# SandeepaInduwaraSamaranayake/SwinVox

Measured on AMD Instinct MI355X. Metric: views/sec fwd+bwd SwinVox-T 224^2, 32^3 voxel, n_views=8, higher is better.
Workload: dtype bf16; 1 GPU; SwinVox-T full pipeline (ResNet50[:layer3] || Swin multi-stage, cross-view attention, decoder, merger, refiner), fwd+2xBCE+bwd, train mode, B=64 samples x V=8 views of 224x224 per GPU; global_batch=64, n_views=8, images_per_gpu=512, parallelism=single GPU, launch=eager (one host launch per kernel, three streams)

## Files before the change

### include/swinvox_hip.h

```cpp
#ifndef SWINVOX_HIP_H
#define SWINVOX_HIP_H
#include <stddef.h>
#include <stdint.h>

#ifdef __cplusplus
extern "C" {
#endif

#define SV_OK 0
#define SV_ERR_INVALID (-1)
#define SV_ERR_LAUNCH (-2)

enum { SV_ACT_NONE = 0, SV_ACT_RELU = 1, SV_ACT_GELU = 2, SV_ACT_LRELU = 3 };
#define SV_BN_SLOTS 16
enum { SV_MATH_F32 = 0, SV_MATH_BF16 = 1, SV_MATH_FP8 = 2, SV_MATH_FP8_FULL = 3 };
enum { SV_F32 = 0, SV_BF16 = 1 };

const char* sv_last_error(void);
int sv_version(void);

typedef struct sv_geom {
  int N;
  int Di, Hi, Wi;
  int Do, Ho, Wo;
// ... 44 lines not shown
                        int act_dtype, void* stream);
int sv_linear_fp8_dgrad_supported(int N, int K, const sv_epilogue* e, int math, int act_dtype);
int sv_linear_fp8_wgrad(const void* dyt, const float* sdc, const void* xt, const float* sxc, float* dw, int M, int N, int K, int ldw, int splits,
                        void* stream);
long long sv_linear_fp8_bwd_launches(int which);
int sv_quant_rows_mx_e4m3(const void* src, int src_dtype, int rows, int K, int ld, void* dst_q, int Kp, void* scales_u8, void* stream);
int sv_linear_mxfp8(const void* xq, const void* xs, const void* wq, const void* ws, void* out, int M, int K, int N, const sv_epilogue* e,
                    void* q_out, void* qs_out, int act_dtype, void* stream);
long long sv_linear_mxfp8_launches(void);
long long sv_quant_rows_mx_launches(void);
int sv_quant_cols_mx_e4m3(const void* src, int src_dtype, int M, int C, int ld, void* dst_q, int Mp, void* scales_u8, float* colsum, void* stream);
int sv_linear_mxfp8_dgrad(const void* dq, const void* ds, const void* wtq, const void* wts, void* dx, int M, int N, int K, const sv_epilogue* e,
                          int act_dtype, void* stream);
size_t sv_linear_mxfp8_wgrad_workspace_floats(int M, int N, int K, int splits);
int sv_linear_mxfp8_wgrad(const void* dyt, const void* dys, const void* xt, const void* xs, float* dw, int M, int N, int K, int ldw, int splits,
                          float* workspace, void* stream);
long long sv_linear_mxfp8_bwd_launches(int which);
long long sv_quant_cols_mx_launches(void);
int sv_mx_rows_to_cols(const void* xq, int Kp, const void* xs, int M, int K, void* dst_q, int Mp, void* scales_u8, void* stream);
long long sv_mx_rows_to_cols_launches(void);
int sv_quant_rows_cols_mx_e4m3(const void* src, int src_dtype, int M, int N, int ld, void* row_q, int Np, void* row_s, void* col_q, int Mp,
                               void* col_s, float* colsum, void* stream);
long long sv_quant_rows_cols_mx_launches(void);
int sv_stencil3_fwd(const void* x, int ldx, int cin_load, int groups, const void* w_bf16, int ntiles16,
                    const float* bias, void* out, int ldc, int col_off, int cout, const void* residual, int ldr,
                    double* stats, int I, int D, int H, int W, long long x_plane_stride, long long out_plane_stride, int act_dtype,
                    void* stream);
size_t sv_stencil3_wgrad_workspace_floats(int cout, int cin);
int sv_stencil3_wgrad(const void* x, int ldx, int cin_load, int groups, const void* dy, int lddy, int cout_load,
                      float* dw, float* dbias, float* workspace, int cout, int cin, int c_stride, int c_valid, int I, int D, int H, int W,
                      long long x_plane_stride, int act_dtype, void* stream);
int sv_tconv4s2_fwd(const void* x, const void* w_packed, const float* bias, void* out, double* stats, int I, int D, int H, int W,
                    int cin, int cout, void* stream);
int sv_pack_weight(const float* src, void* dst, int A, int B, int T, int swap, int pad_to, int out_dtype, void* stream);
typedef struct sv_pack_desc {
  const float* src; void* dst;
  int A, B, T, swap, rows_out, inner_out, block0, reserved;
} sv_pack_desc;
int sv_pack_weights_block_elems(void);
int sv_pack_weights(const sv_pack_desc* descs_dev, int n, int total_blocks, int out_dtype, void* stream);
int sv_colsum(const void* x, int rows, int cols, int ld, float* out, int accumulate, int act_dtype, void* stream);
int sv_cast(const void* src, int src_dtype, void* dst, int dst_dtype, long long n, void* stream);

int sv_layernorm_fwd(const void* x, const float* gamma, const float* beta, void* y, float* mean, float* rstd,
                     long long rows, int C, float eps, int merge_H, int merge_W, int act_dtype, void* stream);
int sv_layernorm_quant_fwd(const void* x, const float* gamma, const float* beta, void* y, float* mean, float* rstd,
                           void* q, int Kp, float* scales, long long rows, int C, float eps, int merge_H, int merge_W,
                           int act_dtype, void* stream);
long long sv_layernorm_quant_launches(void);
int sv_layernorm_quant_mx_fwd(const void* x, const float* gamma, const float* beta, void* y, float* mean, float* rstd,
                              void* q, int Kp, void* scales_u8, long long rows, int C, float eps,
                              int merge_H, int merge_W, int act_dtype, void* stream);
long long sv_layernorm_quant_mx_launches(void);
size_t sv_layernorm_bwd_workspace_floats(int C);
int sv_layernorm_bwd(const void* dy, const void* x, const float* gamma, const float* mean, const float* rstd,
                     void* dx, float* dgamma, float* dbeta, float* workspace, long long rows, int C, int merge_H, int merge_W,
                     int accumulate_dx, int act_dtype, void* stream);
size_t sv_ln_image_workspace_floats(int I, int L);
int sv_ln_image_fwd(const void* x, const float* w, const float* b, void* y, float* meanrstd, float* workspace,
                    int I, int L, float eps, float drop_p, uint32_t seed, const uint32_t* seed_epoch, int act_dtype, void* stream);
int sv_ln_image_bwd(const void* dy, const void* x, const float* w, const float* meanrstd, void* dx, float* dw,
                    float* db, double* sums_ws , int I, int L, float drop_p, uint32_t seed,
                    const uint32_t* seed_epoch, int act_dtype, void* stream);
int sv_bn_stats(const void* x, long long M, int C, int ld, double* sums, int act_dtype, void* stream);
int sv_bn_finalize(const double* sums, long long count, const float* gamma, const float* beta, float* running_mean,
                   float* running_var, float momentum, float eps, int training, float* scale, float* shift,
// ... 127 lines not shown
```

### swinvox_amd/csrc/stencil.hip

```cpp
#include "common.h"
#include <map>
#include <mutex>
#include <type_traits>

namespace sv {

constexpr int TZ = 4, TY = 8, TX = 8;
constexpr int HZ = TZ + 2, HY = TY + 2, HX = TX + 2;
constexpr int HPOS = HZ * HY * HX;
constexpr int NVOX = TZ * TY * TX;
typedef __attribute__((address_space(3))) bf16x4 lds_bf16x4_t;

__device__ __forceinline__ bf16x4 to_bf16x4(float4 v) {
  bf16x4 b;
  b[0] = (__bf16)v.x; b[1] = (__bf16)v.y; b[2] = (__bf16)v.z; b[3] = (__bf16)v.w;
  return b;
}
__device__ __forceinline__ bf16x4 to_bf16x4(bf16x4 v) { return v; }

__device__ __forceinline__ int xcd_first_tile() {
  const int n = gridDim.x, b = blockIdx.x;
  return (n & 7) == 0 ? (b & 7) * (n >> 3) + (b >> 3) : b;
}

// ... 420 lines not shown
          for (int j = 0; j < 4; ++j) o[j] = (__bf16)(acc[j] + bias4[j]);
          const int oz = 2 * jz + az, oy = 2 * jy + ay, ox = 2 * xx + ax;
          *reinterpret_cast<bf16x4*>(Os + ((oz * 8 + oy) * 16 + ox) * 8 + lg * 4) = o;
        }
      }
    }
    __syncthreads();
#pragma unroll
    for (int k = 0; k < 4; ++k) {
      const int v = tid + 256 * k;
      const int ox = v & 15, oy = (v >> 4) & 7, oz = v >> 7;
      const bf16x8 o = *reinterpret_cast<const bf16x8*>(Os + v * 8);
      const size_t pos = (((size_t)img * (2 * p.D) + 2 * z0 + oz) * (2 * p.H) + 2 * y0 + oy) * (2 * p.W) + 2 * x0 + ox;
      *reinterpret_cast<bf16x8*>(p.out + pos * 8) = o;
      if (p.stats) {
#pragma unroll
        for (int c = 0; c < 8; ++c) { const double f = (double)(float)o[c]; st1[c] += f; st2[c] += f * f; }
      }
    }
    __syncthreads();
  }
  if (p.stats) {
#pragma unroll
    for (int c = 0; c < 8; ++c) {
      float a = (float)st1[c], b2 = (float)st2[c];
      a = wave_sum(a); b2 = wave_sum(b2);
      if (lane == 0) { red[wave][c] = a; red[wave][8 + c] = b2; }
    }
    __syncthreads();
    if (tid < 16 && (tid & 7) < p.cout) {
      const float v = red[0][tid] + red[1][tid] + red[2][tid] + red[3][tid];
      double* st = p.stats + (size_t)(blockIdx.x % SV_BN_SLOTS) * 2 * p.cout;
      atomicAdd(st + (tid >> 3) * p.cout + (tid & 7), (double)v);
    }
  }
}

}

using namespace sv;

static int resident_per_cu(const void* kernel, int threads = 256) {
  static std::mutex mu;
  static std::map<const void*, int> cache;
  std::lock_guard<std::mutex> lk(mu);
  auto it = cache.find(kernel);
  if (it != cache.end()) return it->second;
  int n = 0;
  if (hipOccupancyMaxActiveBlocksPerMultiprocessor(&n, kernel, threads, 0) != hipSuccess || n < 1) { (void)hipGetLastError(); n = 1; }
  cache[kernel] = n;
  return n;
}

static int stencil_check(int I, int D, int H, int W) {
  SV_REQUIRE(I > 0 && D % 8 == 0 && H % TY == 0 && W % TX == 0, "stencil3: grid %dx%dx%d must be a multiple of the 8x8x8 brick", D, H, W);
  return SV_OK;
}

#define SV_STENCIL_LAUNCH(GG, NTT, VV)                                                                                     \
  do {                                                                                                                    \
    constexpr int nthr = StencilBrickF<GG>::NTHR;                                                                         \
    const int nt_ = I * (D / StencilBrickF<GG>::TZV) * (H / TY) * (W / TX);                                               \
    a.ntiles = nt_;                                                                                                       \
    const int resident = 256 * resident_per_cu((const void*)stencil3_fwd_kernel<GG, NTT, AT, VV>, nthr);                  \
    hipLaunchKernelGGL((stencil3_fwd_kernel<GG, NTT, AT, VV>), dim3(nt_ < resident ? nt_ : resident), dim3(nthr), 0, s, a); \
  } while (0)
// ... 35 lines not shown

extern "C" size_t sv_stencil3_wgrad_workspace_floats(int cout, int cin) { return (size_t)WG_SLOTS * cout * cin * 27; }

extern "C" int sv_stencil3_wgrad(const void* x, int ldx, int cin_load, int groups, const void* dy, int lddy, int cout_load,
                                 float* dw, float* dbias, float* workspace, int cout, int cin, int c_stride, int c_valid, int I, int D, int H,
                                 int W, long long x_plane_stride, int act_dtype, void* stream) {
  SV_REQUIRE(x && dy && dw, "stencil3_wgrad: null argument");
  SV_REQUIRE(x_plane_stride >= 0 && x_plane_stride % 4 == 0 && (!x_plane_stride || cin_load % ldx == 0), "stencil3_wgrad: bad plane stride");
  SV_REQUIRE_ACT(act_dtype);
  if (int rc = stencil_check(I, D, H, W)) return rc;
  SV_REQUIRE(cin_load % 4 == 0 && cin_load <= 16 * groups && ldx % 4 == 0 && cout_load % 4 == 0 && cout_load <= 16 && lddy % 4 == 0,
             "stencil3_wgrad: bad channel layout");
  SV_REQUIRE(cout > 0 && cout <= 16 && cin > 0 && c_stride > 0 && c_valid > 0, "stencil3_wgrad: bad channel counts");
  SV_REQUIRE((((uintptr_t)x | (uintptr_t)dy) & (act_dtype == SV_BF16 ? 7 : 15)) == 0, "stencil3_wgrad: operands must be aligned to 4 elements");
  SV_REQUIRE(groups == 1 || groups == 3, "stencil3_wgrad: unsupported groups=%d", groups);
    const int ntiles = I * (D / (groups == 3 ? StencilBrick<3>::TZV : StencilBrick<1>::TZV)) * (H / TY) * (W / TX);
  hipStream_t s = (hipStream_t)stream;
  SV_DISPATCH_ACT(act_dtype,
    const int per_cu = groups == 1 ? resident_per_cu((const void*)stencil3_wgrad_kernel<1, AT>, StencilBrick<1>::NTHR)
                                   : resident_per_cu((const void*)stencil3_wgrad_kernel<3, AT>, StencilBrick<3>::NTHR);
    const int resident = 256 * per_cu;
    const int blocks = ntiles < resident ? ntiles : resident;
    StencilWArgsT<AT> a{static_cast<const AT*>(x), ldx, cin_load, x_plane_stride, static_cast<const AT*>(dy), lddy, cout_load, dw, workspace, dbias, cout, cin, c_stride, c_valid,
                        I, D, H, W, ntiles};
    if (groups == 1) hipLaunchKernelGGL((stencil3_wgrad_kernel<1, AT>), dim3(blocks), dim3(StencilBrick<1>::NTHR), 0, s, a);
    else hipLaunchKernelGGL((stencil3_wgrad_kernel<3, AT>), dim3(blocks), dim3(StencilBrick<3>::NTHR), 0, s, a););
  if (workspace) hipLaunchKernelGGL(stencil_wgrad_fold_kernel, dim3(cdiv(cout * cin * 27, 256)), dim3(256), 0, s, workspace, dw, cout * cin * 27);
  return check_launch("sv_stencil3_wgrad");
}

extern "C" int sv_tconv4s2_fwd(const void* x, const void* w_packed, const float* bias, void* out, double* stats, int I, int D, int H, int W,
                               int cin, int cout, void* stream) {
  SV_REQUIRE(x && w_packed && out && I > 0, "tconv4s2_fwd: null argument");
  SV_REQUIRE(cin == 32 && cout > 0 && cout <= 8, "tconv4s2_fwd: built for 32 input and <= 8 output channels (got %d -> %d)", cin, cout);
  SV_REQUIRE(D % T4_JZ == 0 && H % T4_JY == 0 && W % T4_JX == 0, "tconv4s2_fwd: input grid %dx%dx%d must be a multiple of the 4x4x8 brick", D, H, W);
  SV_REQUIRE((((uintptr_t)x | (uintptr_t)w_packed | (uintptr_t)out) & 15) == 0, "tconv4s2_fwd: operands must be 16-byte aligned");
  TConv4Args a{static_cast<const __bf16*>(x), static_cast<const __bf16*>(w_packed), bias, static_cast<__bf16*>(out), stats, cout, I, D, H, W,
               I * (D / T4_JZ) * (H / T4_JY) * (W / T4_JX)};
  const int blocks = a.nbricks < 512 ? a.nbricks : 512;
  hipLaunchKernelGGL(tconv4s2_fwd_kernel, dim3(blocks), dim3(256), 0, (hipStream_t)stream, a);
  return check_launch("sv_tconv4s2_fwd");
}
```

### swinvox_amd/hip.py

```python
from __future__ import annotations

import ctypes as C
import os
import threading

import torch

_HERE = os.path.dirname(os.path.abspath(__file__))
LIB_PATH = os.environ.get("SV_HIP_LIB") or os.path.join(_HERE, "libswinvox_hip.so")

ACT_NONE, ACT_RELU, ACT_GELU, ACT_LRELU = 0, 1, 2, 3
MATH_F32, MATH_BF16, MATH_FP8, MATH_FP8_FULL = 0, 1, 2, 3
F32, BF16 = 0, 1


class Geom(C.Structure):
    _fields_ = [(n, C.c_int) for n in ("N", "Di", "Hi", "Wi", "Do", "Ho", "Wo", "Ci", "Co", "kd", "kh", "kw",
                                        "sd", "sh", "sw", "pd", "ph", "pw", "ldi")]


class Epilogue(C.Structure):
    _fields_ = [("bias", C.c_void_p), ("residual", C.c_void_p), ("ldr", C.c_int), ("row_scale", C.c_void_p),
                ("rows_per_scale", C.c_int), ("pre_act", C.c_void_p), ("stats", C.c_void_p), ("act", C.c_int),
                ("slope", C.c_float), ("act_grad_src", C.c_void_p), ("act_grad_kind", C.c_int), ("ldc", C.c_int),
# ... 27 lines not shown
    "sv_conv_gather": (_I, [_P, _P, _P, C.POINTER(Geom), C.POINTER(Epilogue), _I]),
    "sv_tconv_gather": (_I, [_P, _P, _P, C.POINTER(Geom), C.POINTER(Epilogue), _I]),
    "sv_conv_gather_is_wide": (_I, None, [_P, _P, _P, C.POINTER(Geom), C.POINTER(Epilogue), _I, _I]),
    "sv_conv_wgrad_is_wide": (_I, None, [_P, _I, _P, C.POINTER(Geom), _I, _I, _I]),
    "sv_conv_wgrad_workspace_floats": (C.c_size_t, None, [C.POINTER(Geom)]),
    "sv_conv_wgrad": (_I, [_P, _I, _P, _P, C.POINTER(Geom), _I, _P, _P, _I]),
    "sv_quant_rows_e4m3": (_I, [_P, _I, _I, _I, _I, _P, _I, _P]),
    "sv_linear_fp8": (_I, [_P, _P, _P, _P, _P, _I, _I, _I, C.POINTER(Epilogue)]),
    "sv_linear_fp8_supported": (_I, None, [_I, _I, C.POINTER(Epilogue), _I, _I]),
    "sv_linear_fp8_launches": (_L, None),
    "sv_quant_cols_e4m3": (_I, [_P, _I, _I, _I, _I, _P, _I, _P, _P]),
    "sv_linear_fp8_dgrad": (_I, [_P, _P, _P, _P, _P, _I, _I, _I, C.POINTER(Epilogue)]),
    "sv_linear_fp8_dgrad_supported": (_I, None, [_I, _I, C.POINTER(Epilogue), _I, _I]),
    "sv_linear_fp8_wgrad": (_I, [_P, _P, _P, _P, _P, _I, _I, _I, _I, _I]),
    "sv_linear_fp8_bwd_launches": (_L, None, [_I]),
    "sv_quant_rows_mx_e4m3": (_I, [_P, _I, _I, _I, _I, _P, _I, _P]),
    "sv_linear_mxfp8": (_I, [_P, _P, _P, _P, _P, _I, _I, _I, C.POINTER(Epilogue), _P, _P]),
    "sv_linear_mxfp8_launches": (_L, None),
    "sv_quant_rows_mx_launches": (_L, None),
    "sv_quant_cols_mx_e4m3": (_I, [_P, _I, _I, _I, _I, _P, _I, _P, _P]),
    "sv_linear_mxfp8_dgrad": (_I, [_P, _P, _P, _P, _P, _I, _I, _I, C.POINTER(Epilogue)]),
    "sv_linear_mxfp8_wgrad_workspace_floats": (C.c_size_t, None, [_I, _I, _I, _I]),
    "sv_linear_mxfp8_wgrad": (_I, [_P, _P, _P, _P, _P, _I, _I, _I, _I, _I, _P]),
    "sv_linear_mxfp8_bwd_launches": (_L, None, [_I]),
    "sv_quant_cols_mx_launches": (_L, None),
    "sv_mx_rows_to_cols": (_I, [_P, _I, _P, _I, _I, _P, _I, _P]),
    "sv_mx_rows_to_cols_launches": (_L, None),
    "sv_quant_rows_cols_mx_e4m3": (_I, [_P, _I, _I, _I, _I, _P, _I, _P, _P, _I, _P, _P]),
    "sv_quant_rows_cols_mx_launches": (_L, None),
    "sv_stencil3_fwd": (_I, [_P, _I, _I, _I, _P, _I, _P, _P, _I, _I, _I, _P, _I, _P, _I, _I, _I, _I, _L, _L]),
    "sv_stencil3_wgrad_workspace_floats": (C.c_size_t, None, [_I, _I]),
    "sv_stencil3_wgrad": (_I, [_P, _I, _I, _I, _P, _I, _I, _P, _P, _P, _I, _I, _I, _I, _I, _I, _I, _I, _L]),
    "sv_tconv4s2_fwd": (_I, [_P, _P, _P, _P, _P, _I, _I, _I, _I, _I, _I]),
    "sv_pack_weight": (_I, [_P, _P, _I, _I, _I, _I, _I, _I]),
    "sv_pack_weights_block_elems": (_I, None),
    "sv_pack_weights": (_I, [_P, _I, _I, _I]),
    "sv_colsum": (_I, [_P, _I, _I, _I, _P, _I]),
    "sv_cast": (_I, [_P, _I, _P, _I, _L]),
    "sv_layernorm_fwd": (_I, [_P, _P, _P, _P, _P, _P, _L, _I, _F, _I, _I]),
    "sv_layernorm_quant_fwd": (_I, [_P, _P, _P, _P, _P, _P, _P, _I, _P, _L, _I, _F, _I, _I]),
    "sv_layernorm_quant_launches": (_L, None),
    "sv_layernorm_quant_mx_fwd": (_I, [_P, _P, _P, _P, _P, _P, _P, _I, _P, _L, _I, _F, _I, _I]),
    "sv_layernorm_quant_mx_launches": (_L, None),
    "sv_layernorm_bwd_workspace_floats": (C.c_size_t, None, [_I]),
    "sv_layernorm_bwd": (_I, [_P, _P, _P, _P, _P, _P, _P, _P, _P, _L, _I, _I, _I, _I]),
    "sv_bn_bwd_workspace_doubles": (C.c_size_t, None, [_I]),
    "sv_ln_image_workspace_floats": (C.c_size_t, None, [_I, _I]),
    "sv_ln_image_fwd": (_I, [_P, _P, _P, _P, _P, _P, _I, _I, _F, _F, _U, _P]),
    "sv_ln_image_bwd": (_I, [_P, _P, _P, _P, _P, _P, _P, _P, _I, _I, _F, _U, _P]),
    "sv_bn_stats": (_I, [_P, _L, _I, _I, _P]),
    "sv_bn_finalize": (_I, [_P, _L, _P, _P, _P, _P, _F, _F, _I, _P, _P, _P, _P, _I]),
    "sv_scale_shift_act": (_I, [_P, _I, _P, _P, _P, _I, _P, _I, _L, _I, _I, _F]),
    "sv_bn_bwd": (_I, [_P, _I, _P, _I, _P, _I, _P, _P, _P, _L, _I, _I, _F, _I, _P, _I, _P, _I, _P, _P, _P, _P, _P]),
    "sv_bn_signs_supported": (_I, None, [_I]),
    "sv_scale_shift_act_signs": (_I, [_P, _I, _P, _P, _P, _I, _P, _I, _L, _I, _I, _F, _P]),
    "sv_bn_bwd_signs": (_I, [_P, _I, _P, _P, _I, _P, _P, _P, _L, _I, _I, _F, _I, _P, _I, _P, _I, _P, _P, _P]),
    "sv_window_attention_fwd": (_I, [_P, _P, _P, _I, _I, _I, _I, _I, _I, _I]),
    "sv_window_attention_fwd_mxq": (_I, [_P, _P, _P, _I, _I, _I, _I, _I, _I, _I, _P, _I, _P]),
    "sv_window_attention_bwd_workspace_floats": (C.c_size_t, None, [_I]),
    "sv_window_attention_windows_per_group": (_I, None, [_I, _I, _I, _I, _I, _I]),
    "sv_window_attention_bwd": (_I, [_P, _P, _P, _P, _P, _P, _I, _I, _I, _I, _I, _I, _I]),
    "sv_stem_space_to_depth": (_I, [_P, _P, _I]),
    "sv_bn_act_maxpool_fwd": (_I, [_P, _P, _P, _P, _P, _I, _I, _I, _I, _I, _F]),
    "sv_bn_maxpool_bwd": (_I, [_P, _P, _P, _P, _P, _P, _P, _P, _I, _I, _I, _I, _I, _F, _I, _P, _P, _P, _P]),
    "sv_bn_act_maxpool3d_fwd": (_I, [_P, _P, _P, _P, _P, _I, _I, _I, _I, _I, _I, _F]),
    "sv_bn_maxpool3d_bwd": (_I, [_P, _P, _P, _P, _P, _P, _P, _P, _I, _I, _I, _I, _I, _I, _F, _I, _P, _P, _P, _P]),
# ... 200 lines not shown
```

### swinvox_amd/ops.py

```python
from __future__ import annotations

import ctypes as C
import threading
from dataclasses import dataclass
from typing import Optional, Tuple

import torch

from . import hip
from .hip import ACT_GELU, ACT_LRELU, ACT_NONE, ACT_RELU, Epilogue, Geom, call, ptr

_STATE = {"math": hip.MATH_F32, "store": torch.float32}


class _CallContext(threading.local):
    packs = None
    arena = None
    awg = None
    bn_tick = None
    dyq = None


_CTX = _CallContext()
BN_SLOTS = 16
BN_BWD_SLOTS, LN_BWD_SLOTS = 16, 32


def set_math(mode: str) -> None:
    _STATE["math"] = {"f32": hip.MATH_F32, "fp32": hip.MATH_F32, "bf16": hip.MATH_BF16}[mode]
    if _STATE["math"] == hip.MATH_F32:
        set_storage("f32")


def get_math() -> str:
    return "bf16" if _STATE["math"] == hip.MATH_BF16 else "f32"
# ... 122 lines not shown

    def pack_fwd(self, w: torch.Tensor) -> torch.Tensor:
        return self._pack(w, "f")

    def pack_dgrad(self, w: torch.Tensor) -> torch.Tensor:
        return self._pack(w, "d")

    def _geom(self, n, gathered_grid, produced_grid, ci, co, ldi) -> Geom:
        return Geom(n, *gathered_grid, *produced_grid, ci, co, *self.k, *self.s, *self.p, ldi)

    def _traced(self, name, n, in_grid, *args):
        tr = hip.TRACE
        if tr is None or name not in tr.names:
            return call(name, *args)
        og = self.out_grid(in_grid)
        if self.transposed:
            pairs = n * in_grid[0] * in_grid[1] * in_grid[2] * self.taps
        else:
            pairs = n * og[0] * og[1] * og[2] * self.taps
        flops = 2.0 * pairs * self.cin * self.cout
        nin, nout = n * in_grid[0] * in_grid[1] * in_grid[2], n * og[0] * og[1] * og[2]
        esz = 2.0 if _STATE["store"] == torch.bfloat16 else 4.0
        nbytes = esz * (nin * self.cin + nout * self.cout) + 4.0 * self.taps * self.cin * self.cout
        tr.begin(name, flops, nbytes, tag=f"n={n} grid={in_grid} cin={self.cin} cout={self.cout} k={self.k} s={self.s} t={int(self.transposed)}")
        call(name, *args)
        tr.end()

    def _halo_tconv(self, in_grid, ldi, ldc, epi) -> bool:
        return (self.transposed and self.k == (4, 4, 4) and self.s == (2, 2, 2) and self.p == (1, 1, 1) and self.cin == 32
                and self.cin_mem == 32 and self.cout == 8 and _STATE["store"] == torch.bfloat16 and _STATE["math"] != hip.MATH_F32
                and ldi in (None, 32) and ldc in (None, 8) and not (set(epi) - {"bias", "stats"})
                and in_grid[0] % 4 == 0 and in_grid[1] % 4 == 0 and in_grid[2] % 8 == 0)

    def forward(self, x, n, in_grid, w_packed, out, *, ldi=None, ldc=None, **epi):
        og = self.out_grid(in_grid)
        if isinstance(w_packed, torch.nn.Parameter) or w_packed.dtype != _STATE["store"]:
            w_packed = self.pack_fwd(w_packed)
        if self._halo_tconv(in_grid, ldi, ldc, epi):
            self._traced("sv_tconv4s2_fwd", n, in_grid, ptr(x), ptr(w_packed), ptr(epi.get("bias")), ptr(out), ptr(epi.get("stats")),
                         n, *in_grid, self.cin, self.cout)
            return og
        g = self._geom(n, in_grid, og, self.cin_mem, self.cout, ldi or self.cin_mem)
        e = _epilogue(ldc or self.cout, **epi)
        self._traced("sv_tconv_gather" if self.transposed else "sv_conv_gather", n, in_grid, ptr(x), ptr(w_packed), ptr(out),
                     C.byref(g), C.byref(e), _STATE["math"])
        return og

    def dgrad(self, dy, n, in_grid, w_dgrad, dx, *, lddy=None, lddx=None, **epi):
        og = self.out_grid(in_grid)
        g = self._geom(n, og, in_grid, self.cout_mem, self.cin, lddy or self.cout_mem)
        e = _epilogue(lddx or self.cin_mem, **epi)
        dense = self.taps == 1 and self.s == (1, 1, 1) and self.p == (0, 0, 0)
        self._traced("sv_conv_gather" if (self.transposed or dense) else "sv_tconv_gather", n, in_grid, ptr(dy), ptr(w_dgrad), ptr(dx),
                     C.byref(g), C.byref(e), _STATE["math"])

    def wgrad(self, dy, x, n, in_grid, dw, *, lddy=None, ldx=None, db=None, async_ok=True):
        aw = _CTX.awg
        if aw is not None and async_ok:
            cur = torch.cuda.current_stream()
            aw.stream.wait_stream(cur)
            aw.held.append((dy, x))
            with torch.cuda.stream(aw.stream):
                self._wgrad(dy, x, n, in_grid, dw, lddy, ldx, db)
            return
        self._wgrad(dy, x, n, in_grid, dw, lddy, ldx, db)

    def _wgrad(self, dy, x, n, in_grid, dw, lddy, ldx, db):
        og = self.out_grid(in_grid)
        if self.transposed:
            g = self._geom(n, og, in_grid, self.cout_mem, self.cin, lddy or self.cout_mem)
            ws = fempty(self.cin * self.taps * self.cout_mem, like=dw) if self.taps > 1 else None
            self._traced("sv_conv_wgrad", n, in_grid, ptr(x), ldx or self.cin_mem, ptr(dy), ptr(dw), C.byref(g), self.cout, ptr(ws),
                         None, _STATE["math"])
            if db is not None:
                colsum(dy, n * og[0] * og[1] * og[2], self.cout, lddy or self.cout_mem, db)
        else:
            g = self._geom(n, in_grid, og, self.cin_mem, self.cout, ldx or self.cin_mem)
            ws = fempty(self.cout * self.taps * self.cin_mem, like=dw) if self.taps > 1 else None
            self._traced("sv_conv_wgrad", n, in_grid, ptr(dy), lddy or self.cout_mem, ptr(x), ptr(dw), C.byref(g), self.cin, ptr(ws),
                         ptr(db), _STATE["math"])


def pack_one(spec: "ConvSpec", w: torch.Tensor, kind: str) -> torch.Tensor:
    A, B, T, swap, pad, rows, inner = spec.pack_args(kind)
    out = torch.empty(rows * T * inner, dtype=_STATE["store"], device=w.device)
    call("sv_pack_weight", ptr(w), ptr(out), A, B, T, swap, pad, hip.ACT)
    return out


class PackCache:

    def __init__(self):
        self.tables = {}
        self.w8 = {}
        self.w8t = {}
        self.w8mx = {}
        self.w8mxt = {}

    def __deepcopy__(self, memo):
        return PackCache()

# ... 657 lines not shown
def _bn_signs_on() -> bool:
    import os
    return _STATE.get("bn_signs", os.environ.get("SV_BN_SIGNS", "1") != "0")


def set_bn_signs(on: bool) -> None:
    _STATE["bn_signs"] = bool(on)


def input_prep_enabled() -> bool:
    import os
    return _STATE.get("input_prep", os.environ.get("SV_INPUT_PREP", "1") != "0")


def set_input_prep(on: bool) -> None:
    _STATE["input_prep"] = bool(on)


def bn_pool_fused_enabled() -> bool:
    import os
    return _STATE.get("bn_pool_fused", os.environ.get("SV_BN_POOL_FUSED", "1") != "0")


def set_bn_pool_fused(on: bool) -> None:
    _STATE["bn_pool_fused"] = bool(on)


def set_conv_halo(mode: int) -> None:
    rc = hip.load().sv_set_conv_halo(int(mode))
    if rc != 0:
        raise RuntimeError(f"sv_set_conv_halo failed (rc={rc}): {hip.load().sv_last_error().decode()}")


def set_conv_halo_wgrad(mode: int) -> None:
    rc = hip.load().sv_set_conv_halo_wgrad(int(mode))
    if rc != 0:
        raise RuntimeError(f"sv_set_conv_halo_wgrad failed (rc={rc}): {hip.load().sv_last_error().decode()}")


def set_bn_probe(fn) -> None:
    _STATE["bn_probe"] = fn


def transpose(src, dst, batch, R, Cc, lds=None, ldd=None, sb=None, db=None):
    lds = lds or Cc
    ldd = ldd or R
    assert src.dtype == dst.dtype
    call("sv_transpose", ptr(src), ptr(dst), batch, R, Cc, lds, ldd, sb if sb is not None else R * lds, db if db is not None else Cc * ldd,
         act=hip.BF16 if src.dtype == torch.bfloat16 else hip.F32)
```

Baseline: 4865 views/s.

## Add halo-brick MFMA kernels for tconv4s2 dgrad/wgrad and 64->32 forward

Adds specialised brick-tiled MFMA kernels for the 4x4x4 stride-2 transposed conv backward pass (dgrad, and wgrad with per-block workspace plus a fold kernel) for 32->8 channels. It also adds a 64->32 forward variant. The backward kernels are enabled by default when the layer shape matches and the brick count passes a threshold. The forward 64 path sits behind an environment flag that defaults off. The intent is to replace generic gather-based backward convolutions in the decoder with LDS-halo-reuse kernels, at the cost of extra workspace and a separate reduction pass.

```diff
diff --git a/include/swinvox_hip.h b/include/swinvox_hip.h
--- a/include/swinvox_hip.h
+++ b/include/swinvox_hip.h
@@ -100,6 +100,10 @@
                       long long x_plane_stride, int act_dtype, void* stream);
 int sv_tconv4s2_fwd(const void* x, const void* w_packed, const float* bias, void* out, double* stats, int I, int D, int H, int W,
                     int cin, int cout, void* stream);
+int sv_tconv4s2_dgrad(const void* dy, const void* w_dgrad, void* dx, int I, int D, int H, int W, int cin, int cout, void* stream);
+size_t sv_tconv4s2_wgrad_workspace_floats(int I, int D, int H, int W);
+int sv_tconv4s2_wgrad(const void* x, const void* dy, float* dw, float* workspace, int I, int D, int H, int W, int cin, int cout,
+                      void* stream);
 int sv_pack_weight(const float* src, void* dst, int A, int B, int T, int swap, int pad_to, int out_dtype, void* stream);
 typedef struct sv_pack_desc {
   const float* src; void* dst;
diff --git a/swinvox_amd/csrc/stencil.hip b/swinvox_amd/csrc/stencil.hip
--- a/swinvox_amd/csrc/stencil.hip
+++ b/swinvox_amd/csrc/stencil.hip
@@ -476,6 +476,336 @@
       const float v = red[0][tid] + red[1][tid] + red[2][tid] + red[3][tid];
       double* st = p.stats + (size_t)(blockIdx.x % SV_BN_SLOTS) * 2 * p.cout;
       atomicAdd(st + (tid >> 3) * p.cout + (tid & 7), (double)v);
+    }
+  }
+}
+
+struct Brick4 { int img, z0, y0, x0; };
+__device__ __forceinline__ Brick4 brick4_of(int t, int D, int H, int W) {
+  const int by = H / T4_JY, bx = W / T4_JX, bz = D / T4_JZ;
+  Brick4 r;
+  r.x0 = (t % bx) * T4_JX; t /= bx; r.y0 = (t % by) * T4_JY; t /= by; r.z0 = (t % bz) * T4_JZ; r.img = t / bz;
+  return r;
+}
+constexpr int T6_PITCH = 72;
+constexpr int T6_NV = (T4_HPOS * 8 + 511) / 512;
+__global__ __launch_bounds__(512, 1) void tconv4s2_fwd64_kernel(const TConv4Args p) {
+  __shared__ __attribute__((aligned(16))) __bf16 Xs[T4_HPOS * T6_PITCH];
+  __shared__ __attribute__((aligned(16))) __bf16 Os[8 * 8 * 16 * 32];
+  __shared__ double red[8][64];
+  const int tid = threadIdx.x, lane = tid & 63, wave = tid >> 6;
+  const int lr = lane & 15, lg = lane >> 4, yy = lr >> 3, xx = lr & 7;
+  const int az = wave >> 2, ay = (wave >> 1) & 1, ax = wave & 1;
+  bf16x8 b[16][2];
+#pragma unroll
+  for (int s = 0; s < 16; ++s) {
+    const int t = s >> 1, dz = t >> 2, dy = (t >> 1) & 1, dx = t & 1;
+    const int kz = az ? 2 - 2 * dz : 3 - 2 * dz, ky = ay ? 2 - 2 * dy : 3 - 2 * dy, kx = ax ? 2 - 2 * dx : 3 - 2 * dx;
+#pragma unroll
+    for (int nb = 0; nb < 2; ++nb)
+      b[s][nb] = *reinterpret_cast<const bf16x8*>(p.w + ((size_t)((lr >> 2) * 8 + nb * 4 + (lr & 3)) * 64 + (kz * 4 + ky) * 4 + kx) * 64 + (s & 1) * 32 + lg * 8);
+  }
+  float bias8[8];
+#pragma unroll
+  for (int j = 0; j < 8; ++j) bias8[j] = p.bias ? p.bias[lg * 8 + j] : 0.f;
+  if (tid < 64) {
+#pragma unroll
+    for (int w = 0; w < 8; ++w) red[w][tid] = 0.0;
+  }
+  bf16x8 hr[T6_NV];
+  auto load_halo = [&](const Brick4& t) {
+#pragma unroll
+    for (int k = 0; k < T6_NV; ++k) {
+      const int i = tid + 512 * k, h = i >> 3, c8 = (i & 7) * 8;
+      const int hx = h % T4_HX; const int t2 = h / T4_HX; const int hy = t2 % T4_HY; const int hz = t2 / T4_HY;
+      const int z = t.z0 - 1 + hz, y = t.y0 - 1 + hy, x = t.x0 - 1 + hx;
+      bf16x8 v = VecN<__bf16, 8>::zero();
+      if (i < T4_HPOS * 8 && (unsigned)z < (unsigned)p.D && (unsigned)y < (unsigned)p.H && (unsigned)x < (unsigned)p.W)
+        v = *reinterpret_cast<const bf16x8*>(p.x + ((((size_t)t.img * p.D + z) * p.H + y) * p.W + x) * 64 + c8);
+      hr[k] = v;
+    }
+  };
+  auto store_halo = [&]() {
+#pragma unroll
+    for (int k = 0; k < T6_NV; ++k) {
+      const int i = tid + 512 * k;
+      if (i < T4_HPOS * 8) *reinterpret_cast<bf16x8*>(Xs + (i >> 3) * T6_PITCH + (i & 7) * 8) = hr[k];
+    }
+  };
+  int brick = blockIdx.x;
+  Brick4 t = brick4_of(brick < p.nbricks ? brick : 0, p.D, p.H, p.W);
+  if (brick < p.nbricks) { load_halo(t); store_halo(); }
+  __syncthreads();
+  const __bf16* arow = Xs + (((az * T4_HY) + yy + ay) * T4_HX + xx + ax) * T6_PITCH + lg * 8;
+  for (; brick < p.nbricks; brick += gridDim.x) {
+    const int next = brick + gridDim.x;
+    Brick4 tn = t;
+    if (next < p.nbricks) { tn = brick4_of(next, p.D, p.H, p.W); load_halo(tn); }
+    float st1[8], st2[8];
+#pragma unroll
+    for (int j = 0; j < 8; ++j) { st1[j] = 0.f; st2[j] = 0.f; }
+#pragma unroll 1
+    for (int jz = 0; jz < T4_JZ; ++jz) {
+      f32x4 acc[2][2];
+#pragma unroll
+      for (int gy = 0; gy < 2; ++gy)
+#pragma unroll
+        for (int nb = 0; nb < 2; ++nb) acc[gy][nb] = (f32x4){0.f, 0.f, 0.f, 0.f};
+      const __bf16* ag = arow + jz * (T4_HY * T4_HX * T6_PITCH);
+#pragma unroll
+      for (int s = 0; s < 16; ++s) {
+        const int tt = s >> 1;
+        const int off = (((tt >> 2) * T4_HY + ((tt >> 1) & 1)) * T4_HX + (tt & 1)) * T6_PITCH + (s & 1) * 32;
+#pragma unroll
+        for (int gy = 0; gy < 2; ++gy) {
+          const bf16x8 a = *reinterpret_cast<const bf16x8*>(ag + off + gy * (2 * T4_HX * T6_PITCH));
+          acc[gy][0] = __builtin_amdgcn_mfma_f32_16x16x32_bf16(b[s][0], a, acc[gy][0], 0, 0, 0);
+          acc[gy][1] = __builtin_amdgcn_mfma_f32_16x16x32_bf16(b[s][1], a, acc[gy][1], 0, 0, 0);
+        }
+      }
+#pragma unroll
+      for (int gy = 0; gy < 2; ++gy) {
+        bf16x8 o;
+#pragma unroll
+        for (int j = 0; j < 4; ++j) { o[j] = (__bf16)(acc[gy][0][j] + bias8[j]); o[4 + j] = (__bf16)(acc[gy][1][j] + bias8[4 + j]); }
+#pragma unroll
+        for (int j = 0; j < 8; ++j) { const float f = (float)o[j]; st1[j] += f; st2[j] += f * f; }
+        const int oz = 2 * jz + az, oy = 2 * (2 * gy + yy) + ay, ox = 2 * xx + ax;
+        *reinterpret_cast<bf16x8*>(Os + ((oz * 8 + oy) * 16 + ox) * 32 + lg * 8) = o;
+      }
+    }
+    if (p.stats) {
+#pragma unroll
+      for (int j = 0; j < 8; ++j) {
+        st1[j] += dpp_move<0xB1>(st1[j]); st1[j] += dpp_move<0x4E>(st1[j]); st1[j] += dpp_move<0x141>(st1[j]); st1[j] += dpp_move<0x140>(st1[j]);
+        st2[j] += dpp_move<0xB1>(st2[j]); st2[j] += dpp_move<0x4E>(st2[j]); st2[j] += dpp_move<0x141>(st2[j]); st2[j] += dpp_move<0x140>(st2[j]);
+      }
+      if (lr == 0) {
+#pragma unroll
+        for (int j = 0; j < 8; ++j) { red[wave][lg * 8 + j] += (double)st1[j]; red[wave][32 + lg * 8 + j] += (double)st2[j]; }
+      }
+    }
+    __syncthreads();
+#pragma unroll
+    for (int k = 0; k < 8; ++k) {
+      const int i = tid + 512 * k, v = i >> 2, c8 = (i & 3) * 8;
+      const int ox = v & 15, oy = (v >> 4) & 7, oz = v >> 7;
+      const size_t pos = (((size_t)t.img * (2 * p.D) + 2 * t.z0 + oz) * (2 * p.H) + 2 * t.y0 + oy) * (2 * p.W) + 2 * t.x0 + ox;
+      *reinterpret_cast<bf16x8*>(p.out + pos * 32 + c8) = *reinterpret_cast<const bf16x8*>(Os + v * 32 + c8);
+    }
+    if (next < p.nbricks) store_halo();
+    t = tn;
+    __syncthreads();
+  }
+  if (p.stats) {
+    __syncthreads();
+    if (tid < 64) {
+      double a = 0.0;
+#pragma unroll
+      for (int w = 0; w < 8; ++w) a += red[w][tid];
+      atomicAdd(p.stats + (size_t)(blockIdx.x % SV_BN_SLOTS) * 64 + tid, a);
+    }
+  }
+}
+
+struct TConv4BArgs {
+  const __bf16* dy;
+  const __bf16* x;
+  const __bf16* w;
+  __bf16* dx;
+  float* ws;
+  int I, D, H, W, nbricks;
+};
+constexpr int T4B_HZ = 2 * T4_JZ + 2, T4B_HY = 2 * T4_JY + 2, T4B_HX = 2 * T4_JX + 2, T4B_HPOS = T4B_HZ * T4B_HY * T4B_HX;
+constexpr int T4B_NV = (T4B_HPOS + 255) / 256;
+constexpr int T4B_WN = 32 * 8 * 64;
+constexpr int T4B_MAXWG = 512;
+
+struct DyBoxRegs {
+  bf16x8 r[T4B_NV];
+  int off[T4B_NV], face[T4B_NV];
+  __device__ __forceinline__ void init(int H2, int W2, int tid) {
+#pragma unroll
+    for (int k = 0; k < T4B_NV; ++k) {
+      const int h = tid + 256 * k;
+      const int hx = h % T4B_HX; const int t2 = h / T4B_HX; const int hy = t2 % T4B_HY; const int hz = t2 / T4B_HY;
+      face[k] = (hz == 0 ? 1 : 0) | (hz == T4B_HZ - 1 ? 2 : 0) | (hy == 0 ? 4 : 0) | (hy == T4B_HY - 1 ? 8 : 0) | (hx == 0 ? 16 : 0) | (hx == T4B_HX - 1 ? 32 : 0) |
+                (h < T4B_HPOS ? 0 : 64);
+      off[k] = ((hz * H2 + hy) * W2 + hx) * 8;
+    }
+  }
+  __device__ __forceinline__ void load(const __bf16* __restrict__ dy, const Brick4& b, int D, int H, int W) {
+    const int out = (b.z0 == 0 ? 1 : 0) | (b.z0 + T4_JZ == D ? 2 : 0) | (b.y0 == 0 ? 4 : 0) | (b.y0 + T4_JY == H ? 8 : 0) | (b.x0 == 0 ? 16 : 0) | (b.x0 + T4_JX == W ? 32 : 0) | 64;
+    const __bf16* corner = dy + ((((long long)b.img * (2 * D) + 2 * b.z0 - 1) * (2 * H) + 2 * b.y0 - 1) * (2 * W) + 2 * b.x0 - 1) * 8;
+#pragma unroll
+    for (int k = 0; k < T4B_NV; ++k) {
+      bf16x8 q = VecN<__bf16, 8>::zero();
+      if ((face[k] & out) == 0) q = *reinterpret_cast<const bf16x8*>(corner + off[k]);
+      r[k] = q;
+    }
+  }
+  __device__ __forceinline__ void store(__bf16* Ds, int tid) const {
+#pragma unroll
+    for (int k = 0; k < T4B_NV; ++k) {
+      const int h = tid + 256 * k;
+      if (h < T4B_HPOS) *reinterpret_cast<bf16x8*>(Ds + h * 8) = r[k];
+    }
+  }
+};
+
+__global__ __launch_bounds__(256, 2) void tconv4s2_dgrad_kernel(const TConv4BArgs p) {
+  __shared__ __attribute__((aligned(16))) __bf16 Ds[T4B_HPOS * 8];
+  const int tid = threadIdx.x, lane = tid & 63, wave = tid >> 6;
+  const int lr = lane & 15, lg = lane >> 4, yy = lr >> 3, xx = lr & 7;
+  bf16x8 b[16][2];
+#pragma unroll
+  for (int s = 0; s < 16; ++s)
+#pragma unroll
+    for (int nb = 0; nb < 2; ++nb)
+      b[s][nb] = *reinterpret_cast<const bf16x8*>(p.w + ((lr >> 2) * 8 + nb * 4 + (lr & 3)) * 512 + s * 32 + lg * 8);
+  DyBoxRegs br;
+  br.init(2 * p.H, 2 * p.W, tid);
+  int brick = blockIdx.x;
+  Brick4 t = brick4_of(brick < p.nbricks ? brick : 0, p.D, p.H, p.W);
+  if (brick < p.nbricks) { br.load(p.dy, t, p.D, p.H, p.W); br.store(Ds, tid); }
+  __syncthreads();
+  const __bf16* arow = Ds + (((2 * wave) * T4B_HY + 2 * yy) * T4B_HX + 2 * xx + lg) * 8;
+  for (; brick < p.nbricks; brick += gridDim.x) {
+    const int next = brick + gridDim.x;
+    Brick4 tn = t;
+    if (next < p.nbricks) { tn = brick4_of(next, p.D, p.H, p.W); br.load(p.dy, tn, p.D, p.H, p.W); }
+    f32x4 acc[2][2];
+#pragma unroll
+    for (int gi = 0; gi < 2; ++gi)
+#pragma unroll
+      for (int nb = 0; nb < 2; ++nb) acc[gi][nb] = (f32x4){0.f, 0.f, 0.f, 0.f};
+#pragma unroll
+    for (int s = 0; s < 16; ++s) {
+      const int kz = s >> 2, ky = s & 3;
+#pragma unroll
+      for (int gi = 0; gi < 2; ++gi) {
+        const bf16x8 a = *reinterpret_cast<const bf16x8*>(arow + ((kz * T4B_HY + 4 * gi + ky) * T4B_HX) * 8);
+        acc[gi][0] = __builtin_amdgcn_mfma_f32_16x16x32_bf16(b[s][0], a, acc[gi][0], 0, 0, 0);
+        acc[gi][1] = __builtin_amdgcn_mfma_f32_16x16x32_bf16(b[s][1], a, acc[gi][1], 0, 0, 0);
+      }
+    }
+#pragma unroll
+    for (int gi = 0; gi < 2; ++gi) {
+      bf16x8 o;
+#pragma unroll
+      for (int j = 0; j < 4; ++j) { o[j] = (__bf16)acc[gi][0][j]; o[4 + j] = (__bf16)acc[gi][1][j]; }
+      const size_t pos = (((size_t)t.img * p.D + t.z0 + wave) * p.H + t.y0 + 2 * gi + yy) * p.W + t.x0 + xx;
+      *reinterpret_cast<bf16x8*>(p.dx + pos * 32 + lg * 8) = o;
+    }
+    t = tn;
+    __syncthreads();
+    if (next < p.nbricks) br.store(Ds, tid);
+    __syncthreads();
+  }
+}
+
+__global__ __launch_bounds__(256, 2) void tconv4s2_wgrad_kernel(const TConv4BArgs p) {
+  __shared__ __attribute__((aligned(16))) __bf16 Ds[T4B_HPOS * 8];
+  __shared__ __attribute__((aligned(16))) __bf16 Xs[T4_JZ * T4_JY * T4_JX * 32];
+  const int tid = threadIdx.x, lane = tid & 63, wave = tid >> 6;
+  const int lr = lane & 15, lg = lane >> 4, q = lr >> 2, pp = lr & 3;
+  f32x4 acc[4][2][2];
+#pragma unroll
+  for (int ky = 0; ky < 4; ++ky)
+#pragma unroll
+    for (int mb = 0; mb < 2; ++mb)
+#pragma unroll
+      for (int nb = 0; nb < 2; ++nb) acc[ky][mb][nb] = (f32x4){0.f, 0.f, 0.f, 0.f};
+  DyBoxRegs br;
+  br.init(2 * p.H, 2 * p.W, tid);
+  bf16x8 xr[2];
+  auto load_x = [&](const Brick4& t) {
+#pragma unroll
+    for (int k = 0; k < 2; ++k) {
+      const int i = tid + 256 * k, v = i >> 2, c8 = (i & 3) * 8;
+      const int ix = v & 7, iy = (v >> 3) & 3, iz = v >> 5;
+      xr[k] = *reinterpret_cast<const bf16x8*>(p.x + ((((size_t)t.img * p.D + t.z0 + iz) * p.H + t.y0 + iy) * p.W + t.x0 + ix) * 32 + c8);
+    }
+  };
+  auto store_x = [&]() {
+#pragma unroll
+    for (int k = 0; k < 2; ++k) *reinterpret_cast<bf16x8*>(Xs + (tid + 256 * k) * 8) = xr[k];
+  };
+  int brick = blockIdx.x;
+  if (brick < p.nbricks) {
+    const Brick4 t = brick4_of(brick, p.D, p.H, p.W);
+    br.load(p.dy, t, p.D, p.H, p.W); load_x(t);
+    br.store(Ds, tid); store_x();
+  }
+  __syncthreads();
+  const __bf16* xsrc = Xs + ((lg * T4_JX) + q) * 32 + pp * 4;
+  const __bf16* dsrc = Ds + (((wave * T4B_HY) + 2 * lg) * T4B_HX + 2 * q + (pp >> 1)) * 8 + (pp & 1) * 4;
+  for (; brick < p.nbricks; brick += gridDim.x) {
+    const int next = brick + gridDim.x;
+    if (next < p.nbricks) {
+      const Brick4 t = brick4_of(next, p.D, p.H, p.W);
+      br.load(p.dy, t, p.D, p.H, p.W); load_x(t);
+    }
+#pragma unroll
+    for (int iz = 0; iz < T4_JZ; ++iz) {
+      bf16x8 a[2];
+#pragma unroll
+      for (int mb = 0; mb < 2; ++mb) {
+        const __bf16* s = xsrc + iz * (T4_JY * T4_JX * 32) + mb * 16;
+        const bf16x4 lo = __builtin_amdgcn_ds_read_tr16_b64_v4bf16((lds_bf16x4_t*)(s));
+        const bf16x4 hi = __builtin_amdgcn_ds_read_tr16_b64_v4bf16((lds_bf16x4_t*)(s + 4 * 32));
+        a[mb] = __builtin_shufflevector(lo, hi, 0, 1, 2, 3, 4, 5, 6, 7);
+      }
+#pragma unroll
+      for (int ky = 0; ky < 4; ++ky)
+#pragma unroll
+        for (int nb = 0; nb < 2; ++nb) {
+          const __bf16* s = dsrc + ((2 * iz * T4B_HY + ky) * T4B_HX + 2 * nb) * 8;
+          const bf16x4 lo = __builtin_amdgcn_ds_read_tr16_b64_v4bf16((lds_bf16x4_t*)(s));
+          const bf16x4 hi = __builtin_amdgcn_ds_read_tr16_b64_v4bf16((lds_bf16x4_t*)(s + 8 * 8));
+          const bf16x8 bv = __builtin_shufflevector(lo, hi, 0, 1, 2, 3, 4, 5, 6, 7);
+          acc[ky][0][nb] = __builtin_amdgcn_mfma_f32_16x16x32_bf16(a[0], bv, acc[ky][0][nb], 0, 0, 0);
+          acc[ky][1][nb] = __builtin_amdgcn_mfma_f32_16x16x32_bf16(a[1], bv, acc[ky][1][nb], 0, 0, 0);
+        }
+    }
+    __syncthreads();
+    if (next < p.nbricks) { br.store(Ds, tid); store_x(); }
+    __syncthreads();
+  }
+  float* dst = p.ws + (size_t)blockIdx.x * T4B_WN + wave * 4096 + lane;
+#pragma unroll
+  for (int ky = 0; ky < 4; ++ky)
+#pragma unroll
+    for (int mb = 0; mb < 2; ++mb)
+#pragma unroll
+      for (int nb = 0; nb < 2; ++nb)
+#pragma unroll
+        for (int j = 0; j < 4; ++j) dst[((ky * 2 + mb) * 2 + nb) * 256 + j * 64] = acc[ky][mb][nb][j];
+}
+
+__global__ __launch_bounds__(1024) void tconv4s2_wgrad_fold_kernel(const float* __restrict__ ws, float* __restrict__ dw, int nslots) {
+  __shared__ float2 part[16][64];
+  const int lane = threadIdx.x & 63, sg = threadIdx.x >> 6;
+  const int e0 = blockIdx.x * 128 + lane * 2;
+  float2 a = make_float2(0.f, 0.f);
+#pragma unroll 4
+  for (int sl = sg; sl < nslots; sl += 16) {
+    const float2 v = *reinterpret_cast<const float2*>(ws + (size_t)sl * T4B_WN + e0);
+    a.x += v.x; a.y += v.y;
+  }
+  part[sg][lane] = a;
+  __syncthreads();
+  if (sg == 0) {
+    float2 v = part[0][lane];
+#pragma unroll
+    for (int w = 1; w < 16; ++w) { v.x += part[w][lane].x; v.y += part[w][lane].y; }
+#pragma unroll
+    for (int h = 0; h < 2; ++h) {
+      const int e = e0 + h;
+      const int al = e & 63, jj = (e >> 6) & 3, nb = (e >> 8) & 1, mb = (e >> 9) & 1, ky = (e >> 10) & 3, kz = e >> 12;
+      const int lr = al & 15, lg = al >> 4;
+      const int ci = 16 * mb + 4 * lg + jj, kx = 2 * nb + (lr >> 3), co = lr & 7;
+      dw[(ci * 8 + co) * 64 + (kz * 4 + ky) * 4 + kx] += h ? v.y : v.x;
     }
   }
 }
@@ -577,12 +907,57 @@
 extern "C" int sv_tconv4s2_fwd(const void* x, const void* w_packed, const float* bias, void* out, double* stats, int I, int D, int H, int W,
                                int cin, int cout, void* stream) {
   SV_REQUIRE(x && w_packed && out && I > 0, "tconv4s2_fwd: null argument");
-  SV_REQUIRE(cin == 32 && cout > 0 && cout <= 8, "tconv4s2_fwd: built for 32 input and <= 8 output channels (got %d -> %d)", cin, cout);
+  SV_REQUIRE((cin == 32 && cout > 0 && cout <= 8) || (cin == 64 && cout == 32),
+             "tconv4s2_fwd: built for 32 input and <= 8 output channels, or 64 -> 32 (got %d -> %d)", cin, cout);
   SV_REQUIRE(D % T4_JZ == 0 && H % T4_JY == 0 && W % T4_JX == 0, "tconv4s2_fwd: input grid %dx%dx%d must be a multiple of the 4x4x8 brick", D, H, W);
   SV_REQUIRE((((uintptr_t)x | (uintptr_t)w_packed | (uintptr_t)out) & 15) == 0, "tconv4s2_fwd: operands must be 16-byte aligned");
   TConv4Args a{static_cast<const __bf16*>(x), static_cast<const __bf16*>(w_packed), bias, static_cast<__bf16*>(out), stats, cout, I, D, H, W,
                I * (D / T4_JZ) * (H / T4_JY) * (W / T4_JX)};
+  SV_REQUIRE((long long)I * (D / T4_JZ) * (H / T4_JY) * (W / T4_JX) < (1ll << 30), "tconv4s2_fwd: too many bricks");
+  if (cin == 64) {
+    SV_REQUIRE(!bias || ((uintptr_t)bias & 3) == 0, "tconv4s2_fwd: bias must be 4-byte aligned");
+    hipLaunchKernelGGL(tconv4s2_fwd64_kernel, dim3(a.nbricks < 256 ? a.nbricks : 256), dim3(512), 0, (hipStream_t)stream, a);
+    return check_launch("sv_tconv4s2_fwd");
+  }
   const int blocks = a.nbricks < 512 ? a.nbricks : 512;
   hipLaunchKernelGGL(tconv4s2_fwd_kernel, dim3(blocks), dim3(256), 0, (hipStream_t)stream, a);
   return check_launch("sv_tconv4s2_fwd");
 }
+
+static int tconv4s2_bwd_check(const char* what, int I, int D, int H, int W, int cin, int cout) {
+  SV_REQUIRE(I > 0, "%s: null argument", what);
+  SV_REQUIRE(cin == 32 && cout == 8, "%s: built for 32 input and 8 output channels (got %d -> %d)", what, cin, cout);
+  SV_REQUIRE(D > 0 && H > 0 && W > 0 && D % T4_JZ == 0 && H % T4_JY == 0 && W % T4_JX == 0, "%s: input grid %dx%dx%d must be a multiple of the 4x4x8 brick", what, D, H, W);
+  SV_REQUIRE((long long)I * (D / T4_JZ) * (H / T4_JY) * (W / T4_JX) < (1ll << 30), "%s: too many bricks", what);
+  return SV_OK;
+}
+
+extern "C" int sv_tconv4s2_dgrad(const void* dy, const void* w_dgrad, void* dx, int I, int D, int H, int W, int cin, int cout, void* stream) {
+  SV_REQUIRE(dy && w_dgrad && dx, "tconv4s2_dgrad: null argument");
+  if (int rc = tconv4s2_bwd_check("tconv4s2_dgrad", I, D, H, W, cin, cout)) return rc;
+  SV_REQUIRE((((uintptr_t)dy | (uintptr_t)w_dgrad | (uintptr_t)dx) & 15) == 0, "tconv4s2_dgrad: operands must be 16-byte aligned");
+  TConv4BArgs a{static_cast<const __bf16*>(dy), nullptr, static_cast<const __bf16*>(w_dgrad), static_cast<__bf16*>(dx), nullptr, I, D, H, W,
+                I * (D / T4_JZ) * (H / T4_JY) * (W / T4_JX)};
+  const int blocks = a.nbricks < T4B_MAXWG ? a.nbricks : T4B_MAXWG;
+  hipLaunchKernelGGL(tconv4s2_dgrad_kernel, dim3(blocks), dim3(256), 0, (hipStream_t)stream, a);
+  return check_launch("sv_tconv4s2_dgrad");
+}
+
+extern "C" size_t sv_tconv4s2_wgrad_workspace_floats(int I, int D, int H, int W) {
+  if (I <= 0 || D <= 0 || H <= 0 || W <= 0) return 0;
+  const long long nb = (long long)I * (D / T4_JZ) * (H / T4_JY) * (W / T4_JX);
+  return (size_t)(nb < T4B_MAXWG ? nb : T4B_MAXWG) * T4B_WN;
+}
+
+extern "C" int sv_tconv4s2_wgrad(const void* x, const void* dy, float* dw, float* workspace, int I, int D, int H, int W, int cin, int cout,
+                                 void* stream) {
+  SV_REQUIRE(x && dy && dw && workspace, "tconv4s2_wgrad: null argument");
+  if (int rc = tconv4s2_bwd_check("tconv4s2_wgrad", I, D, H, W, cin, cout)) return rc;
+  SV_REQUIRE((((uintptr_t)x | (uintptr_t)dy) & 15) == 0 && ((uintptr_t)dw & 3) == 0 && ((uintptr_t)workspace & 7) == 0, "tconv4s2_wgrad: x and dy must be 16-byte aligned (the workspace to 8 bytes)");
+  TConv4BArgs a{static_cast<const __bf16*>(dy), static_cast<const __bf16*>(x), nullptr, nullptr, workspace, I, D, H, W,
+                I * (D / T4_JZ) * (H / T4_JY) * (W / T4_JX)};
+  const int blocks = a.nbricks < T4B_MAXWG ? a.nbricks : T4B_MAXWG;
+  hipLaunchKernelGGL(tconv4s2_wgrad_kernel, dim3(blocks), dim3(256), 0, (hipStream_t)stream, a);
+  hipLaunchKernelGGL(tconv4s2_wgrad_fold_kernel, dim3(T4B_WN / 128), dim3(1024), 0, (hipStream_t)stream, workspace, dw, blocks);
+  return check_launch("sv_tconv4s2_wgrad");
+}
diff --git a/swinvox_amd/hip.py b/swinvox_amd/hip.py
--- a/swinvox_amd/hip.py
+++ b/swinvox_amd/hip.py
@@ -83,6 +83,9 @@
     "sv_stencil3_wgrad_workspace_floats": (C.c_size_t, None, [_I, _I]),
     "sv_stencil3_wgrad": (_I, [_P, _I, _I, _I, _P, _I, _I, _P, _P, _P, _I, _I, _I, _I, _I, _I, _I, _I, _L]),
     "sv_tconv4s2_fwd": (_I, [_P, _P, _P, _P, _P, _I, _I, _I, _I, _I, _I]),
+    "sv_tconv4s2_dgrad": (_I, [_P, _P, _P, _I, _I, _I, _I, _I, _I]),
+    "sv_tconv4s2_wgrad_workspace_floats": (C.c_size_t, None, [_I, _I, _I, _I]),
+    "sv_tconv4s2_wgrad": (_I, [_P, _P, _P, _P, _I, _I, _I, _I, _I, _I]),
     "sv_pack_weight": (_I, [_P, _P, _I, _I, _I, _I, _I, _I]),
     "sv_pack_weights_block_elems": (_I, None),
     "sv_pack_weights": (_I, [_P, _I, _I, _I]),
diff --git a/swinvox_amd/ops.py b/swinvox_amd/ops.py
--- a/swinvox_amd/ops.py
+++ b/swinvox_amd/ops.py
@@ -1,6 +1,7 @@
 from __future__ import annotations
 
 import ctypes as C
+import os
 import threading
 from dataclasses import dataclass
 from typing import Optional, Tuple
@@ -189,11 +190,26 @@
                 and ldi in (None, 32) and ldc in (None, 8) and not (set(epi) - {"bias", "stats"})
                 and in_grid[0] % 4 == 0 and in_grid[1] % 4 == 0 and in_grid[2] % 8 == 0)
 
+    def _halo_tconv64(self, n, in_grid, ldi, ldc, epi) -> bool:
+        mode = _STATE["tconv_halo"] if _STATE["tconv_halo_fwd64"] else 0
+        if mode == 0 or not (self.transposed and self.k == (4, 4, 4) and self.s == (2, 2, 2) and self.p == (1, 1, 1) and self.cin == 64
+                             and self.cin_mem == 64 and self.cout == 32 and _STATE["store"] == torch.bfloat16 and _STATE["math"] != hip.MATH_F32
+                             and ldi in (None, 64) and ldc in (None, 32) and not (set(epi) - {"bias", "stats"})
+                             and in_grid[0] % 4 == 0 and in_grid[1] % 4 == 0 and in_grid[2] % 8 == 0):
+            return False
+        return mode == 2 or n * (in_grid[0] // 4) * (in_grid[1] // 4) * (in_grid[2] // 8) >= TCONV_HALO_MIN_BRICKS
+
+    def _halo_tconv_bwd(self, n, in_grid, ldi, ldc) -> bool:
+        mode = _STATE["tconv_halo"]
+        if mode == 0 or self.cout_mem != 8 or not self._halo_tconv(in_grid, ldi, ldc, {}):
+            return False
+        return mode == 2 or n * (in_grid[0] // 4) * (in_grid[1] // 4) * (in_grid[2] // 8) >= TCONV_HALO_MIN_BRICKS
+
     def forward(self, x, n, in_grid, w_packed, out, *, ldi=None, ldc=None, **epi):
         og = self.out_grid(in_grid)
         if isinstance(w_packed, torch.nn.Parameter) or w_packed.dtype != _STATE["store"]:
             w_packed = self.pack_fwd(w_packed)
-        if self._halo_tconv(in_grid, ldi, ldc, epi):
+        if self._halo_tconv(in_grid, ldi, ldc, epi) or self._halo_tconv64(n, in_grid, ldi, ldc, epi):
             self._traced("sv_tconv4s2_fwd", n, in_grid, ptr(x), ptr(w_packed), ptr(epi.get("bias")), ptr(out), ptr(epi.get("stats")),
                          n, *in_grid, self.cin, self.cout)
             return og
@@ -205,6 +221,9 @@
 
     def dgrad(self, dy, n, in_grid, w_dgrad, dx, *, lddy=None, lddx=None, **epi):
         og = self.out_grid(in_grid)
+        if not epi and self._halo_tconv_bwd(n, in_grid, lddx, lddy):
+            self._traced("sv_tconv4s2_dgrad", n, in_grid, ptr(dy), ptr(w_dgrad), ptr(dx), n, *in_grid, self.cin, self.cout)
+            return
         g = self._geom(n, og, in_grid, self.cout_mem, self.cin, lddy or self.cout_mem)
         e = _epilogue(lddx or self.cin_mem, **epi)
         dense = self.taps == 1 and self.s == (1, 1, 1) and self.p == (0, 0, 0)
@@ -224,6 +243,12 @@
 
     def _wgrad(self, dy, x, n, in_grid, dw, lddy, ldx, db):
         og = self.out_grid(in_grid)
+        if self._halo_tconv_bwd(n, in_grid, ldx, lddy):
+            ws = fempty(int(hip.load().sv_tconv4s2_wgrad_workspace_floats(n, *in_grid)), like=dw)
+            self._traced("sv_tconv4s2_wgrad", n, in_grid, ptr(x), ptr(dy), ptr(dw), ptr(ws), n, *in_grid, self.cin, self.cout)
+            if db is not None:
+                colsum(dy, n * og[0] * og[1] * og[2], self.cout, 8, db)
+            return
         if self.transposed:
             g = self._geom(n, og, in_grid, self.cout_mem, self.cin, lddy or self.cout_mem)
             ws = fempty(self.cin * self.taps * self.cout_mem, like=dw) if self.taps > 1 else None
@@ -947,6 +972,30 @@
         raise RuntimeError(f"sv_set_conv_halo failed (rc={rc}): {hip.load().sv_last_error().decode()}")
 
 
+TCONV_HALO_MIN_BRICKS = 128
+_STATE["tconv_halo"] = 1
+_STATE["tconv_halo_fwd64"] = os.environ.get("SV_TCONV_HALO_FWD64", "0") == "1"
+
+
+def set_tconv_halo(mode: int) -> None:
+    mode = int(mode)
+    if mode not in (0, 1, 2):
+        raise RuntimeError(f"set_tconv_halo: mode must be 0, 1 or 2 (got {mode})")
+    _STATE["tconv_halo"] = mode
+
+
+def set_tconv_halo_fwd64(on: bool) -> None:
+    _STATE["tconv_halo_fwd64"] = bool(on)
+
+
+def get_tconv_halo() -> int:
+    return _STATE["tconv_halo"]
+
+
+if os.environ.get("SV_TCONV_HALO", "") != "":
+    set_tconv_halo(int(os.environ["SV_TCONV_HALO"]))
+
+
 def set_conv_halo_wgrad(mode: int) -> None:
     rc = hip.load().sv_set_conv_halo_wgrad(int(mode))
     if rc != 0:
```

Result: no change. 4901 views/s (median of 6 runs) (+0.7%).
